# apirrone/Open_Duck_Playground

Measured on AMD Instinct MI355X. Metric: env-steps/sec open_duck_mini_v2 flat_terrain @8192 envs; 1/2/4/8-GPU scaling, higher is better.
Workload: dtype f32

## Files before the change

include/odk.h:

```cpp
#ifndef ODK_H
#define ODK_H

#include <stdint.h>

#ifdef __cplusplus
extern "C" {
#endif

typedef struct odk_model odk_model;
typedef struct odk_batch odk_batch;

enum odk_status {
  ODK_OK = 0,
  ODK_ERR_INVALID = -1,
  ODK_ERR_UNSUPPORTED = -2,
  ODK_ERR_HIP = -3,
  ODK_ERR_NOMEM = -4
};

#define ODK_NOBS 101
#define ODK_NPRIV 212
#define ODK_NOBS_STANDING 85
#define ODK_NPRIV_STANDING 153
#define ODK_ENV_JOYSTICK 0
// ... 28 lines not shown
  float* metrics_dev;
} odk_outputs;

enum odk_param {
  ODK_PARAM_BODY_MASS = 0,
  ODK_PARAM_BODY_IPOS_TORSO = 1,
  ODK_PARAM_DOF_FRICTIONLOSS = 2,
  ODK_PARAM_DOF_ARMATURE = 3,
  ODK_PARAM_QPOS0 = 4,
  ODK_PARAM_KP = 5
};

const char* odk_last_error(void);
void odk_default_config(odk_env_config* cfg);
void odk_default_config_standing(odk_env_config* cfg);
void odk_obs_sizes(int env_kind, int* nobs, int* npriv);

int odk_model_load(const void* blob, uint64_t len, odk_model** out);
void odk_model_free(odk_model* m);
int odk_model_dims(const odk_model* m, int* nq, int* nv, int* nu, int* nbody);
int odk_model_obs_sizes(const odk_model* m, int env_kind, int* nobs, int* npriv);

int odk_model_reduced(const odk_model* m, int* paired, int* nvr, int* nMr, int* nHr, int* red_main, int* red_twin);
int odk_model_env_lds_floats(const odk_model* m);

int odk_batch_create(const odk_model* m, const odk_env_config* cfg, int nenv, int device, const float* prm_table,
                     const double* dxs, int nx, const double* dys, int ny, const double* dths, int nth, const double* ranges6,
                     int nsteps_in_period, odk_batch** out);
void odk_batch_destroy(odk_batch* b);
int odk_batch_set_config(odk_batch* b, const odk_env_config* cfg);

int odk_batch_set_param(odk_batch* b, int param, const float* host_values, int count_per_env);

int odk_reset(odk_batch* b, uint32_t seed, uint32_t env_id_offset, const odk_outputs* outs, void* stream);

int odk_step(odk_batch* b, const float* action_dev, const odk_outputs* outs, void* stream);

int odk_batch_bind_commands(odk_batch* b, const float* cmd_dev, int row_stride);

#define ODK_NXTERM 12
enum odk_xterm {
  ODK_XTERM_LIN_VEL_Z = 0, ODK_XTERM_ANG_VEL_XY = 1, ODK_XTERM_ORIENTATION = 2, ODK_XTERM_BASE_HEIGHT = 3, ODK_XTERM_ENERGY = 4,
  ODK_XTERM_JOINT_POS_LIMITS = 5, ODK_XTERM_TERMINATION = 6, ODK_XTERM_POSE = 7, ODK_XTERM_FEET_SLIP = 8, ODK_XTERM_FEET_CLEARANCE = 9,
  ODK_XTERM_FEET_HEIGHT = 10, ODK_XTERM_FEET_AIR_TIME = 11
};
typedef struct {
// ... 148 lines not shown
```

open_duck_playground_amd/csrc/odk_engine.hip:

```cpp
#include <hip/hip_runtime.h>
#include <stddef.h>

#include <cmath>
#include <cstdarg>
#include <cstdio>
#include <cstdlib>
#include <cstring>
#include <array>
#include <string>
#include <vector>

#include "../../include/odk.h"
#include "odk_kernels.h"

using namespace odk;

struct RecLay {
  int CMD, LAST, LAST2, LAST3, MT, AIR, PEAK, PUSH, AHIST, IMU, EPSTEPS, TRUNC, DONE, EPSUM, EPLEN, EPMET, KEY0, KEY1, CTR, STEP, PSTEP, PINT, IMI, LCON, NINFO;
};
constexpr RecLay rec_lay(int nu) {
  RecLay r{};
  r.CMD = 0; r.LAST = 7; r.LAST2 = r.LAST + nu; r.LAST3 = r.LAST2 + nu; r.MT = r.LAST3 + nu; r.AIR = r.MT + nu; r.PEAK = r.AIR + 2; r.PUSH = r.PEAK + 2;
  r.AHIST = r.PUSH + 2; r.IMU = r.AHIST + 3 * nu; r.EPSTEPS = r.IMU + 9; r.TRUNC = r.EPSTEPS + 1; r.DONE = r.TRUNC + 1; r.EPSUM = r.DONE + 1; r.EPLEN = r.EPSUM + 1;
  r.EPMET = r.EPLEN + 1; r.KEY0 = r.EPMET + ODK_NMETRIC; r.KEY1 = r.KEY0 + 1; r.CTR = r.KEY1 + 1; r.STEP = r.CTR + 1; r.PSTEP = r.STEP + 1; r.PINT = r.PSTEP + 1;
// ... 920 lines not shown
  if (solref[1] <= 0) b = -solref[1] / dmax;
  P[0] = k; P[1] = b; P[2] = dmin; P[3] = dmax; P[4] = 1.0f / width; P[5] = mid; P[6] = power;
  P[7] = 1.0f / powf(mid, power - 1.0f); P[8] = 1.0f / powf(1.0f - mid, power - 1.0f);
}

namespace {
struct SparseLayout { int depth[MAXV], adr[MAXV], ancmask[MAXV], descmask[MAXV], anc_at[MAXV][MAXV], nnz; };
void sparse_layout(const int* parent, int n, SparseLayout& L) {
  L.nnz = 0;
  for (int i = 0; i < n; i++) {
    L.depth[i] = parent[i] < 0 ? 0 : L.depth[parent[i]] + 1;
    L.adr[i] = L.nnz; L.nnz += L.depth[i] + 1;
    L.ancmask[i] = 0; L.descmask[i] = 0;
  }
  for (int i = 0; i < n; i++) {
    int a = i;
    for (int c = L.depth[i]; c >= 0; c--, a = parent[a]) {
      L.anc_at[i][c] = a;
      if (a != i) { L.ancmask[i] |= 1 << a; L.descmask[a] |= 1 << i; }
    }
  }
}
}
static void fill_body_st(DevModel& m) {
  auto fill = [&](BodySt& b, int bi, bool in) {
    memset(&b, 0, sizeof(b));
    b.level = in ? m.body_level[bi] : -2;
    b.parent = m.body_parent[bi];
    b.nchild = in ? m.body_nchild[bi] : 0;
    b.pathmask = in ? m.body_pathmask[bi] : 0;
    b.is_path = in ? m.body_is_path[bi] : 0;
    b.upmask = in ? m.body_upmask[bi] : 0;
    b.path_head = in ? m.body_path_head[bi] : 0;
    for (int k = 0; k < 3; k++) b.child[k] = m.body_children[bi][k];
    b.njnt = (in && b.level > 0) ? m.body_jntnum[bi] : 0;
    for (int k = 0; k < 2; k++) {
      const bool on = k < b.njnt;
      const int j = on ? m.body_jntadr[bi] + k : 0;
      b.jj[k] = j;
      b.jd[k] = m.jnt_dofadr[j];
      b.jr[k] = (m.paired && m.dof_tkind[b.jd[k]] == 2) ? -1 : m.dof_red[b.jd[k]];
      for (int c = 0; c < 3; c++) b.ax[k][c] = on ? m.jnt_axis[j][c] : 0.0f;
    }
    for (int c = 0; c < 3; c++) { b.pos[c] = m.body_pos[bi][c]; b.ipos[c] = m.body_ipos[bi][c]; }
    for (int c = 0; c < 4; c++) b.quat[c] = m.body_quat[bi][c];
    for (int c = 0; c < 6; c++) b.inertia[c] = m.body_inertia[bi][c];
  };
  for (int bi = 0; bi < m.nb; bi++) fill(m.body_st[bi], bi, true);
  fill(m.body_st[MAXB], 0, false);
}

static bool build_reduced_tables(DevModel& m) {
  m.paired = 0; m.nrchain = 0;
  int ntwin = 0;
  for (int d = 0; d < MAXV; d++) { m.dof_tkind[d] = 0; m.dof_red[d] = 0; m.red_main[d] = 0; m.red_twin[d] = -1; }
  for (int v = 7; v < m.nv; v++) {
    const int u = v - 1, ju = m.dof_jnt[u], jv = m.dof_jnt[v];
    if (ju < 0 || jv < 0 || m.dof_tkind[u] != 0) continue;
    const bool same = m.dof_body[u] == m.dof_body[v] && m.dof_anc[v][1] == u && m.jnt_axis[ju][0] == m.jnt_axis[jv][0] &&
                      m.jnt_axis[ju][1] == m.jnt_axis[jv][1] && m.jnt_axis[ju][2] == m.jnt_axis[jv][2];
    if (!same) continue;
    m.dof_tkind[u] = 1; m.dof_tkind[v] = 2; ntwin++;
  }
  m.paired = ntwin > 0;
  int nr = 0;
  for (int d = 0; d < m.nv; d++) {
    if (m.dof_tkind[d] == 2) { m.dof_red[d] = m.dof_red[d - 1]; continue; }
    m.dof_red[d] = nr; m.red_main[nr] = d; m.red_twin[nr] = m.dof_tkind[d] == 1 ? d + 1 : -1; nr++;
  }
  m.nvr = nr;
  int rparent[MAXV], rvparent[MAXV];
  for (int r = 0; r < nr; r++) {
// ... 431 lines not shown
  if (eulerdamp != 0 || m.iterations != 1) { delete mo; return fail(ODK_ERR_UNSUPPORTED, "kernels implement iterations=1, eulerdamp=disable (open_duck_mini_v2.xml:6-8)"); }
  for (int s = 0; s < m.nsensor; s++) {
    int b = m.site_body[m.sensor_site[s]];
    bool ok = (b == m.base_body) || (b == m.foot_body[0]) || (b == m.foot_body[1]);
    if (!ok || ((m.sensor_type[s] == 2 || m.sensor_type[s] == 8) && b != m.base_body)) { delete mo; return fail(ODK_ERR_UNSUPPORTED, "sensor %d placement", s); }
  }
  m.np_count = 0;
  for (int b2 = 0; b2 < m.nb; b2++) {
    if (!(m.body_level[b2] >= 0 && m.body_nchild[b2] > 0 && !m.body_is_path[b2])) continue;
    if (m.np_count == 4) { delete mo; return fail(ODK_ERR_UNSUPPORTED, "more than four branching bodies above the serial chains"); }
    const int i = m.np_count++;
    m.np_body[i] = b2; m.np_nsrc[i] = 0;
    for (int c2 = 0; c2 < m.nb; c2++) {
      bool below = false;
      for (int a2 = c2; a2 > 0; a2 = m.body_parent[a2]) if (a2 == b2) { below = true; break; }
      if (!below || m.body_level[c2] < 0) continue;
      if (!m.body_is_path[c2] || m.body_path_head[c2]) {
        if (m.np_nsrc[i] == 6) { delete mo; return fail(ODK_ERR_UNSUPPORTED, "more than six sources in a subtree fold"); }
        m.np_src[i][m.np_nsrc[i]++] = c2;
      }
    }
  }
  if (!build_reduced_tables(m)) { delete mo; return fail(ODK_ERR_UNSUPPORTED, "dof tree is not a floating base with up to three serial chains of <= 5 (twin-merged) dofs"); }
  fill_body_st(m);
  int dt_max = 0, dv_max = 0;
  for (int d = 0; d < m.nv; d++) { dt_max = m.dof_depth[d] > dt_max ? m.dof_depth[d] : dt_max; dv_max = m.vdof_depth[d] > dv_max ? m.vdof_depth[d] : dv_max; }
  mo->shape = -1;
#define X(i, S) if (mo->shape < 0 && m.nq == S::NQ && m.nv == S::NV && m.nb == S::NB && m.nu == S::NU && m.nj == S::NJ && m.nM == S::NM && m.nH == S::NH && m.nrow == S::NROW && \
                    dt_max <= S::DT && dv_max <= S::DV) mo->shape = i;
  ODK_SHAPES(X)
#undef X
  if (mo->shape < 0) {
    const int dtm = dt_max, dvm = dv_max;
    delete mo;
    return fail(ODK_ERR_UNSUPPORTED, "model shape nq=%d nv=%d nb=%d nu=%d nj=%d nM=%d nH=%d nrow=%d depth=%d vdepth=%d has no compiled kernel (tools/new_shape.py <xml> prints the two lines to add to odk_engine.hip)",
                m.nq, m.nv, m.nb, m.nu, m.nj, m.nM, m.nH, m.nrow, dtm, dvm);
  }
  int shape_cl = 5; bool shape_eq = false;
#define X(i, S) if (mo->shape == i) { shape_cl = S::CL; shape_eq = S::EQ; }
  ODK_SHAPES(X)
#undef X
  for (int c = 0; c < m.nrchain; c++)
    if (m.rchain_len[c] > shape_cl) { const int len = m.rchain_len[c]; delete mo; return fail(ODK_ERR_UNSUPPORTED, "a serial chain of %d (twin-merged) dofs: the kernels of this model shape solve chains of <= %d", len, shape_cl); }
  if (!m.floor_is_plane && mo->shape != 1) { delete mo; return fail(ODK_ERR_UNSUPPORTED, "height-field floors are built for the backlash model only"); }

  if (m.cone && m.foot_prim != 0) {
    delete mo; return fail(ODK_ERR_UNSUPPORTED, "<option cone=\"elliptic\">: the elliptic-cone kernels are built for convex (box / mesh) feet, not sphere / capsule feet");
// ... 87 lines not shown
}
extern "C" void odk_model_free(odk_model* m) { delete m; }
extern "C" int odk_model_dims(const odk_model* m, int* nq, int* nv, int* nu, int* nbody) {
  if (!m) return fail(ODK_ERR_INVALID, "null model");
  if (nq) *nq = m->h.nq; if (nv) *nv = m->h.nv; if (nu) *nu = m->h.nu; if (nbody) *nbody = m->h.nb;
  return ODK_OK;
}
extern "C" int odk_model_obs_sizes(const odk_model* m, int env_kind, int* nobs, int* npriv) {
  if (!m) return fail(ODK_ERR_INVALID, "null model");
  obs_sizes_nu(m->h.nu, env_kind, nobs, npriv);
  return ODK_OK;
}

#ifndef ODK_PROFILE
static_assert(EnvL<ShapeA>::wg_floats(2) * sizeof(float) <= 20480, "shape A: LDS image too large for 8 workgroups per CU");
static_assert(EnvL<ShapeB>::wg_floats(2) * sizeof(float) <= 20480, "shape B: LDS image too large for 8 workgroups per CU");
#endif
extern "C" int odk_model_reduced(const odk_model* m, int* paired, int* nvr, int* nMr, int* nHr, int* red_main, int* red_twin) {
  if (!m) return fail(ODK_ERR_INVALID, "null model");
  if (paired) *paired = m->h.paired; if (nvr) *nvr = m->h.nvr; if (nMr) *nMr = m->h.nMr; if (nHr) *nHr = m->h.nHr;
  for (int r = 0; r < m->h.nvr; r++) { if (red_main) red_main[r] = m->h.red_main[r]; if (red_twin) red_twin[r] = m->h.red_twin[r]; }
  return ODK_OK;
}
extern "C" int odk_model_env_lds_floats(const odk_model* m) {
  if (!m) return -1;
#define X(i, S) if (m->shape == i) return EnvL<S>::TOTAL;
  ODK_SHAPES(X)
#undef X
  return -1;
}

template <class S> static void fill_sizes(odk_batch* b) {
  b->rec_size = Rec<S>::SIZE; b->frec_size = Rec<S>::FSIZE; b->lds_total = S::TOTAL; b->dr_size = DRL<S>::SIZE; b->env_lds = EnvL<S>::TOTAL;
}

static void to_dev_cfg(const odk_env_config& c, EnvCfg& d, int nu) {
  d.ctrl_dt = c.ctrl_dt; d.action_scale = c.action_scale; d.dof_vel_scale = c.dof_vel_scale; d.max_motor_velocity = c.max_motor_velocity;
  d.noise_level = c.noise_level; d.noise_gyro = c.noise_gyro; d.noise_accelerometer = c.noise_accelerometer; d.noise_gravity = c.noise_gravity;
  d.noise_joint_vel = c.noise_joint_vel;
  memcpy(d.qpos_noise_scale, c.qpos_noise_scale, sizeof(d.qpos_noise_scale)); memcpy(d.reward_scales, c.reward_scales, sizeof(d.reward_scales));
  d.tracking_sigma = c.tracking_sigma; d.push_enable = c.push_enable;
  memcpy(d.push_interval_range, c.push_interval_range, 8); memcpy(d.push_magnitude_range, c.push_magnitude_range, 8);
  memcpy(d.cmd_range, c.cmd_range, sizeof(d.cmd_range));
  d.use_imitation = c.use_imitation; d.use_motor_speed_limits = c.use_motor_speed_limits; d.autoreset = c.autoreset;
  d.episode_length = c.episode_length; d.n_substeps = c.n_substeps;
  d.kind = c.env_kind; d.reset_base_qvel = c.reset_base_qvel;
// ... 454 lines not shown
```

open_duck_playground_amd/csrc/odk_kernels.h:

```cpp
#pragma once
#include <hip/hip_runtime.h>

#include "odk_model.h"

namespace odk {

#define ODK_SYNC() asm volatile("" ::: "memory")

constexpr float MINVAL_F = 1e-15f;
constexpr float PI_F = 3.14159265358979323846f;

struct EnvCfg {
  float ctrl_dt, action_scale, dof_vel_scale, max_motor_velocity;
  float noise_level, noise_gyro, noise_accelerometer, noise_gravity, noise_joint_vel;
  float qpos_noise_scale[16];
  float reward_scales[7];
  float tracking_sigma;
  float push_enable, push_interval_range[2], push_magnitude_range[2];
  float cmd_range[7][2];
  int use_imitation, use_motor_speed_limits, autoreset, episode_length, n_substeps;
  int kind, nobs, npriv;
  float reset_base_qvel;
};

// ... 92 lines not shown
#endif

#define ODK_DPP(v, ctrl, rmask) __int_as_float(__builtin_amdgcn_update_dpp(0, __float_as_int(v), ctrl, rmask, 0xF, true))
struct OpSum { static __device__ __forceinline__ float f(float a, float b) { return a + b; } };
struct OpMax { static __device__ __forceinline__ float f(float a, float b) { return fmaxf(a, b); } };
struct OpMin { static __device__ __forceinline__ float f(float a, float b) { return fminf(a, b); } };
typedef unsigned int odk_u2 __attribute__((ext_vector_type(2)));
template <int G, class Op> __device__ __forceinline__ float greduce(float v) {
  v = Op::f(v, ODK_DPP(v, 0xB1, 0xF));
  v = Op::f(v, ODK_DPP(v, 0x4E, 0xF));
  v = Op::f(v, ODK_DPP(v, 0x141, 0xF));
  v = Op::f(v, ODK_DPP(v, 0x140, 0xF));
  const unsigned iv = __float_as_uint(v);
  const odk_u2 h = __builtin_amdgcn_permlane16_swap(iv, iv, false, false);
  v = Op::f(__uint_as_float(h[0]), __uint_as_float(h[1]));
  if (G == 64) {
    const unsigned iw = __float_as_uint(v);
    const odk_u2 w = __builtin_amdgcn_permlane32_swap(iw, iw, false, false);
    v = Op::f(__uint_as_float(w[0]), __uint_as_float(w[1]));
  }
  return v;
}
template <int G> __device__ __forceinline__ float gsum(float v) { return greduce<G, OpSum>(v); }
template <int G, int N> __device__ __forceinline__ void gsum_n(float* v) {
  if constexpr (G == 32) {
    float o[N];
#pragma unroll
    for (int i = 0; i < N; i++) {
      float x = v[i];
      x += ODK_DPP(x, 0xB1, 0xF); x += ODK_DPP(x, 0x4E, 0xF); x += ODK_DPP(x, 0x141, 0xF); x += ODK_DPP(x, 0x140, 0xF);
      v[i] = x;
      o[i] = __int_as_float(__builtin_amdgcn_ds_swizzle(__float_as_int(x), 0x401F));
    }
#pragma unroll
    for (int i = 0; i < N; i++) v[i] += o[i];
  } else {
#pragma unroll
    for (int i = 0; i < N; i++) v[i] = gsum<G>(v[i]);
  }
}
__device__ __forceinline__ unsigned fkey(float v) { const unsigned b = __float_as_uint(v); return b ^ ((b >> 31) ? 0xFFFFFFFFu : 0x80000000u); }
__device__ __forceinline__ float fkey_inv(unsigned k) { return __uint_as_float(k ^ ((k >> 31) ? 0x80000000u : 0xFFFFFFFFu)); }
#define ODK_DPPU(v, ctrl) ((unsigned)__builtin_amdgcn_update_dpp(0, (int)(v), ctrl, 0xF, 0xF, true))
template <int G, bool MAX> __device__ __forceinline__ unsigned greduce_u(unsigned v) {
  auto op = [](unsigned a, unsigned b) { return MAX ? (a > b ? a : b) : (a < b ? a : b); };
  v = op(v, ODK_DPPU(v, 0xB1));
// ... 144 lines not shown
      for (int h = 0; h < 2; h++) {
        const int j = 2 * jp + h;
        int off = S::O_CDOF * 4;
        if (j < S::NVR && ((rel >> j) & 1)) off = (S::O_M + (j < r ? st.r_Madr + m->red_depth[j] : m->red_Madr[j] + st.r_depth)) * 4;
        pk |= off << (16 * h);
      }
      st.m_adr[jp] = pk;
    }
  }
  const int i = lane < S::NV ? lane : 0;
  st.d_on = lane < S::NV;
  st.d_body = m->dof_body[i];
  st.d_act = st.d_on ? m->dof_act[i] : -1;
  st.d_flrow = st.d_on ? m->dof_flrow[i] : -1;
  st.d_limrow = st.d_on ? m->dof_limrow[i] : -1;
  st.d_foot = st.d_on ? (m->foot_dofmask[0][i] | (m->foot_dofmask[1][i] << 1)) : 0;
  st.d_damping = m->dof_damping[i];
  st.d_lim_on = st.d_limrow >= 0;
  st.d_qadr = m->dof_qadr[i];
  st.d_lo = m->dof_range[i][0]; st.d_hi = m->dof_range[i][1];
  st.d_tkind = (S::PAIRED && st.d_on) ? m->dof_tkind[i] : 0;
  st.d_red = S::PAIRED ? m->dof_red[i] : i;
}
template <class S>
__device__ __forceinline__ void load_body(BodySt& b, const DevModel* __restrict__ m, int lane) {
  b = m->body_st[lane < S::NB ? lane : MAXB];
}
__device__ __forceinline__ void load_act(ActSt& a, const DevModel* __restrict__ m, int act) {
  const int u = act >= 0 ? act : 0;
  a.bias2 = m->act_bias2[u]; a.clo = m->act_ctrlrange[u][0]; a.chi = m->act_ctrlrange[u][1];
  a.flo = m->act_forcerange[u][0]; a.fhi = m->act_forcerange[u][1];
  a.climited = m->act_ctrllimited[u]; a.flimited = m->act_forcelimited[u];
}
__device__ __forceinline__ void load_fl(FlSt& f, const DevModel* __restrict__ m, int lane) {
  const int r = lane < m->nfl ? lane : 0;
  f.D = m->fl_D[r]; f.R = m->fl_R[r]; f.b = m->fl_b[r]; f.dof = m->fl_dof[r];
}
template <class S, int G>
__device__ __forceinline__ void load_hot(HotSt& h, const DevModel* __restrict__ m, const Statics<S, G>& st, int lane) {
  load_act(h.as, m, st.d_act);
  load_fl(h.fs, m, lane);
  const int f = (lane >> 4) & 1, j = lane & 15;
  const int jv = (lane < 32 && j < m->foot_nvert[f]) ? j : 0;
  for (int k = 0; k < 3; k++) h.vb[k] = m->foot_vert[f][jv][k];
}
__device__ __forceinline__ int load_rent(const DevModel* __restrict__ m, int p, int n) { const int e = m->R_ent[p < n ? p : 0]; return p < n ? e : -1; }
__device__ __forceinline__ int load_rhent(const DevModel* __restrict__ m, int p, int n) { const int e = m->RH_ent[p < n ? p : 0]; return p < n ? e : -1; }

template <int G, int DMAX, int NVT>
// ... 1254 lines not shown
}

template <class S, int G, int HF, bool PRE = false>
__device__ __forceinline__ void forward_env(float* L, const int* RT, const DevModel* __restrict__ m, const float* __restrict__ hfield, const Statics<S, G>& st, int lane, int flags, const HotSt& hot = HotSt()) {
  const float* SH = reinterpret_cast<const float*>(RT);
  const float* CT = SH + S::SH_CT;
  constexpr int NV = S::NV, NB = S::NB, NR = S::NVR;
  using ST = Statics<S, G>;
  float* QPOS = L + S::O_QPOS; float* QVEL = L + S::O_QVEL; float* WARM = L + S::O_WARM; float* CTRL = L + S::O_CTRL;
  float* Q0 = L + S::O_Q0; float* MASS = L + S::O_MASS; float* ARM = L + S::O_ARM; float* FRL = L + S::O_FRL; float* KP = L + S::O_KP;
  float* XPOS = L + S::O_XPOS; float* XQUAT = L + S::O_XQUAT; float* CVEL = L + S::O_CVEL; float* CACC = L + S::O_CACC;
  float* CFRC = L + S::O_CFRC; float* CRB = L + S::O_CRB; float* SC = L + S::O_SC; float* CDOF = L + S::O_CDOF;
  float* BUF6 = L + S::O_BUF6; float* BUF6B = L + S::O_BUF6B; float* M = L + S::O_M; float* HL = L + S::O_HL;
  float* QFS = L + S::O_QFS; float* QAS = L + S::O_QAS; float* X = L + S::O_X; float* MA = L + S::O_MA; float* GRAD = L + S::O_GRAD;
  float* MV = L + S::O_MV; float* ED = L + S::O_D; float* AREF = L + S::O_AREF; float* JAR = L + S::O_JAR; float* JV = L + S::O_JV;
  float* W = L + S::O_W; float* CDIST = L + S::O_CDIST; float* CR = L + S::O_CR; float* SCR = L + S::O_SCR;
  float* SENS = L + S::O_SENS; float* ACTF = L + S::O_ACTF;
  const int nfl = m->nfl, nlim = m->nlim, r0c = nfl + nlim;
  const float dt = m->dt;
  const float ref[3] = {QPOS[0], QPOS[1], QPOS[2]};
  ODK_PROF_BEGIN();

  BodySt bs;
  load_body<S>(bs, m, lane);
  if (st.j_qadr >= 0) {
    float s, c;
    const float x = 0.5f * (QPOS[st.j_qadr] - Q0[st.j_qadr]);
    if (fabsf(x) <= 1.7f) {
      const float x2 = x * x;
      float ps = 1.6059043836821613e-10f, pc = -1.1470745597729725e-11f;
      ps = fmaf(ps, x2, -2.505210838544172e-08f); pc = fmaf(pc, x2, 2.08767569878681e-09f);
      ps = fmaf(ps, x2, 2.7557319223985893e-06f); pc = fmaf(pc, x2, -2.755731922398589e-07f);
      ps = fmaf(ps, x2, -0.0001984126984126984f); pc = fmaf(pc, x2, 2.48015873015873e-05f);
      ps = fmaf(ps, x2, 0.008333333333333333f); pc = fmaf(pc, x2, -0.001388888888888889f);
      ps = fmaf(ps, x2, -0.16666666666666666f); pc = fmaf(pc, x2, 0.041666666666666664f);
      ps = fmaf(ps, x2, 1.0f); pc = fmaf(pc, x2, -0.5f);
      s = ps * x; c = fmaf(pc, x2, 1.0f);
    } else {
      sincosf(x, &s, &c);
    }
    SC[2 * lane] = s; SC[2 * lane + 1] = c;
  }
  ODK_SYNC();
  ODK_PROF(0);
  {
    float p[3] = {0, 0, 0}, q[4] = {1, 0, 0, 0}, cvel[6] = {0, 0, 0, 0, 0, 0}, cacc[6] = {0, 0, 0, 0, 0, 0};
    if (bs.level == -1) {
// ... 35 lines not shown
            if (jj < bs.njnt) {
              float axw[3], cd[6], dot[6];
              qrot(axw, q, bs.ax[jj]);
              const float off[3] = {ref[0] - p[0], ref[1] - p[1], ref[2] - p[2]};
              cd[0] = axw[0]; cd[1] = axw[1]; cd[2] = axw[2];
              cross3(cd + 3, axw, off);
              const int d = bs.jd[jj], col = bs.jr[jj];
              if (col >= 0) {
#pragma unroll
                for (int k = 0; k < 6; k++) CDOF[k * NR + col] = cd[k];
              }
              const float qv = QVEL[d];
              cross_motion(dot, cvel, cd);
#pragma unroll
              for (int k = 0; k < 6; k++) { cacc[k] += dot[k] * qv; cvel[k] += cd[k] * qv; }
              const float s = SC[2 * bs.jj[jj]], c = SC[2 * bs.jj[jj] + 1];
              const float qj[4] = {c, s * bs.ax[jj][0], s * bs.ax[jj][1], s * bs.ax[jj][2]};
              qmul(q, q, qj);
            }
          }
          qnormalize(q);
        }
#pragma unroll
        for (int k = 0; k < 3; k++) XPOS[k * NB + lane] = p[k];
#pragma unroll
        for (int k = 0; k < 4; k++) XQUAT[k * NB + lane] = q[k];
#pragma unroll
        for (int k = 0; k < 6; k++) { CVEL[k * NB + lane] = cvel[k]; CACC[k * NB + lane] = cacc[k]; }
      }
      ODK_SYNC();
    }
    {
      const bool isp = bs.is_path != 0, head = bs.path_head != 0;
      float ql[4] = {bs.quat[0], bs.quat[1], bs.quat[2], bs.quat[3]}, qb[2][4];
#pragma unroll
      for (int jj = 0; jj < 2; jj++) {
#pragma unroll
        for (int k = 0; k < 4; k++) qb[jj][k] = ql[k];
        if (jj < bs.njnt) {
          const float s = SC[2 * bs.jj[jj]], c = SC[2 * bs.jj[jj] + 1];
          const float qj[4] = {c, s * bs.ax[jj][0], s * bs.ax[jj][1], s * bs.ax[jj][2]};
          qmul(ql, ql, qj);
        }
      }
      float tp[3] = {bs.pos[0], bs.pos[1], bs.pos[2]}, tq[4] = {ql[0], ql[1], ql[2], ql[3]};
      float ppq[4] = {1, 0, 0, 0}, pcv[6] = {0, 0, 0, 0, 0, 0}, pca[6] = {0, 0, 0, 0, 0, 0};
      if (isp && head) {
        const int pb = bs.parent;
        float pp[3], t[3];
        for (int k = 0; k < 3; k++) pp[k] = XPOS[k * NB + pb];
        for (int k = 0; k < 4; k++) ppq[k] = XQUAT[k * NB + pb];
        for (int k = 0; k < 6; k++) { pcv[k] = CVEL[k * NB + pb]; pca[k] = CACC[k * NB + pb]; }
        qrot(t, ppq, tp);
        tp[0] = pp[0] + t[0]; tp[1] = pp[1] + t[1]; tp[2] = pp[2] + t[2];
        qmul(tq, ppq, tq);
      }
#pragma unroll
      for (int si = 0; si < 3; si++) {
        float up[3], uq[4];
#pragma unroll
        for (int k = 0; k < 3; k++) up[k] = __shfl_up(tp[k], 1 << si, G);
#pragma unroll
        for (int k = 0; k < 4; k++) uq[k] = __shfl_up(tq[k], 1 << si, G);
        if ((bs.upmask >> si) & 1) {
          float t[3];
          qrot(t, uq, tp);
          tp[0] = up[0] + t[0]; tp[1] = up[1] + t[1]; tp[2] = up[2] + t[2];
          qmul(tq, uq, tq);
        }
      }
      {
        float uq[4];
#pragma unroll
        for (int k = 0; k < 4; k++) uq[k] = __shfl_up(tq[k], 1, G);
        if (isp && !head) { ppq[0] = uq[0]; ppq[1] = uq[1]; ppq[2] = uq[2]; ppq[3] = uq[3]; }
      }
      float cd[2][6], qv[2] = {0, 0}, cinc[6] = {0, 0, 0, 0, 0, 0};
#pragma unroll
      for (int jj = 0; jj < 2; jj++) {
#pragma unroll
        for (int k = 0; k < 6; k++) cd[jj][k] = 0.0f;
        if (isp && jj < bs.njnt) {
          float qw[4], axw[3];
          qmul(qw, ppq, qb[jj]);
          qrot(axw, qw, bs.ax[jj]);
          const float off[3] = {ref[0] - tp[0], ref[1] - tp[1], ref[2] - tp[2]};
          cd[jj][0] = axw[0]; cd[jj][1] = axw[1]; cd[jj][2] = axw[2];
          cross3(cd[jj] + 3, axw, off);
          const int d = bs.jd[jj], col = bs.jr[jj];
          if (col >= 0) {
#pragma unroll
            for (int k = 0; k < 6; k++) CDOF[k * NR + col] = cd[jj][k];
          }
          qv[jj] = QVEL[d];
#pragma unroll
          for (int k = 0; k < 6; k++) cinc[k] += cd[jj][k] * qv[jj];
        }
      }
      float cv[6];
#pragma unroll
      for (int k = 0; k < 6; k++) cv[k] = cinc[k] + pcv[k];
#pragma unroll
      for (int si = 0; si < 3; si++) {
        float u[6];
#pragma unroll
        for (int k = 0; k < 6; k++) u[k] = __shfl_up(cv[k], 1 << si, G);
        const bool ok = (bs.upmask >> si) & 1;
#pragma unroll
        for (int k = 0; k < 6; k++) cv[k] += ok ? u[k] : 0.0f;
      }
      {
        float u[6];
#pragma unroll
        for (int k = 0; k < 6; k++) u[k] = __shfl_up(cv[k], 1, G);
        if (isp && !head) {
#pragma unroll
          for (int k = 0; k < 6; k++) pcv[k] = u[k];
        }
      }
      float ca[6];
#pragma unroll
      for (int k = 0; k < 6; k++) ca[k] = pca[k];
      if (isp) {
        float vb[6] = {pcv[0], pcv[1], pcv[2], pcv[3], pcv[4], pcv[5]};
#pragma unroll
        for (int jj = 0; jj < 2; jj++) {
          if (jj < bs.njnt) {
            float dot[6];
            cross_motion(dot, vb, cd[jj]);
#pragma unroll
            for (int k = 0; k < 6; k++) { ca[k] += dot[k] * qv[jj]; vb[k] += cd[jj][k] * qv[jj]; }
          }
        }
      }
#pragma unroll
      for (int si = 0; si < 3; si++) {
        float u[6];
#pragma unroll
        for (int k = 0; k < 6; k++) u[k] = __shfl_up(ca[k], 1 << si, G);
        const bool ok = (bs.upmask >> si) & 1;
#pragma unroll
        for (int k = 0; k < 6; k++) ca[k] += ok ? u[k] : 0.0f;
      }
      if (isp) {
        qnormalize(tq);
#pragma unroll
        for (int k = 0; k < 3; k++) { p[k] = tp[k]; XPOS[k * NB + lane] = tp[k]; }
#pragma unroll
        for (int k = 0; k < 4; k++) { q[k] = tq[k]; XQUAT[k * NB + lane] = tq[k]; }
#pragma unroll
        for (int k = 0; k < 6; k++) { cvel[k] = cv[k]; cacc[k] = ca[k]; CVEL[k * NB + lane] = cv[k]; CACC[k * NB + lane] = ca[k]; }
      }
      ODK_SYNC();
    }
    float acc[16];
#pragma unroll
    for (int k = 0; k < 16; k++) acc[k] = 0.0f;
    if (lane < NB) {
      if (bs.level < 0) {
#pragma unroll
        for (int k = 0; k < 3; k++) XPOS[k * NB + lane] = p[k];
#pragma unroll
        for (int k = 0; k < 4; k++) XQUAT[k * NB + lane] = q[k];
#pragma unroll
        for (int k = 0; k < 6; k++) { CVEL[k * NB + lane] = 0; CACC[k * NB + lane] = 0; }
      }
      float R[9];
      q2mat(R, q);
      float ip[3] = {bs.ipos[0], bs.ipos[1], bs.ipos[2]};
      {
        const float i0 = L[S::O_IPOS1], i1 = L[S::O_IPOS1 + 1], i2 = L[S::O_IPOS1 + 2];
        asm volatile("" :: "v"(i0), "v"(i1), "v"(i2));
        ip[0] = lane == 1 ? i0 : ip[0]; ip[1] = lane == 1 ? i1 : ip[1]; ip[2] = lane == 1 ? i2 : ip[2];
      }
      float off[3];
      for (int k = 0; k < 3; k++) off[k] = p[k] + R[3 * k] * ip[0] + R[3 * k + 1] * ip[1] + R[3 * k + 2] * ip[2] - ref[k];
      const float* f = bs.inertia;
      const float Ib[9] = {f[0], f[3], f[4], f[3], f[1], f[5], f[4], f[5], f[2]};
      float T[9], Iw[9];
      for (int i = 0; i < 3; i++)
        for (int j = 0; j < 3; j++) T[3 * i + j] = R[3 * i] * Ib[j] + R[3 * i + 1] * Ib[3 + j] + R[3 * i + 2] * Ib[6 + j];
      for (int i = 0; i < 3; i++)
        for (int j = 0; j < 3; j++) Iw[3 * i + j] = T[3 * i] * R[3 * j] + T[3 * i + 1] * R[3 * j + 1] + T[3 * i + 2] * R[3 * j + 2];
      const float mb = MASS[lane], o2 = dot3(off, off);
      float ci[10];
      ci[0] = Iw[0] + mb * (o2 - off[0] * off[0]);
      ci[1] = Iw[4] + mb * (o2 - off[1] * off[1]);
      ci[2] = Iw[8] + mb * (o2 - off[2] * off[2]);
      ci[3] = Iw[1] - mb * off[0] * off[1];
      ci[4] = Iw[2] - mb * off[0] * off[2];
      ci[5] = Iw[5] - mb * off[1] * off[2];
      ci[6] = mb * off[0]; ci[7] = mb * off[1]; ci[8] = mb * off[2];
      ci[9] = mb;
      float fr[6], t1[6], a3[3], c3[3];
      inert_mul(fr, ci, cacc);
      inert_mul(t1, ci, cvel);
      cross3(a3, cvel, t1);
      cross3(c3, cvel + 3, t1 + 3);
      fr[0] += a3[0] + c3[0]; fr[1] += a3[1] + c3[1]; fr[2] += a3[2] + c3[2];
      cross3(a3, cvel, t1 + 3);
      fr[3] += a3[0]; fr[4] += a3[1]; fr[5] += a3[2];
      const bool dyn = bs.level >= 0;
#pragma unroll
      for (int k = 0; k < 10; k++) acc[k] = dyn ? ci[k] : 0.0f;
#pragma unroll
      for (int k = 0; k < 6; k++) acc[10 + k] = dyn ? fr[k] : 0.0f;
    }
    ODK_PROF(1);
#pragma unroll
    for (int si = 0; si < 3; si++) {
      const bool ok = (bs.pathmask >> si) & 1;
      float t[16];
#pragma unroll
      for (int k = 0; k < 16; k++) t[k] = __shfl_down(acc[k], 1 << si, G);
#pragma unroll
      for (int k = 0; k < 16; k++) acc[k] += ok ? t[k] : 0.0f;
    }
    if (lane < NB) {
#pragma unroll
      for (int k = 0; k < 10; k++) CRB[k * NB + lane] = acc[k];
#pragma unroll
      for (int k = 0; k < 6; k++) CFRC[k * NB + lane] = acc[10 + k];
    }
    ODK_SYNC();
  }
  {
    float* ACC = CFRC;
    static_assert(S::O_CRB == S::O_CFRC + 6 * NB, "cfrc | crb must be contiguous");
    const int nnp = m->np_count;
    const int slot = lane >> 4, q = lane & 15;
    float t[2] = {0.0f, 0.0f};
#pragma unroll
    for (int pass = 0; pass < 2; pass++) {
      const int i = pass * (G / 16) + slot;
      if (i < nnp) {
        const int ns = m->np_nsrc[i];
        int src[6];
#pragma unroll
        for (int c = 0; c < 6; c++) src[c] = m->np_src[i][c];
        float x = 0.0f;
#pragma unroll
        for (int c = 0; c < 6; c++) { const float y = ACC[q * NB + src[c]]; x += c < ns ? y : 0.0f; }
        t[pass] = x;
      }
    }
// ... 1133 lines not shown
```

open_duck_playground_amd/csrc/odk_model.h:

```cpp
#pragma once
#include <stdint.h>

namespace odk {

constexpr int EQ_MAX = 2;
constexpr int EQP_MAX = 2, EQP_ROWS = 9;
constexpr int MAXV = 32;
constexpr int MAXQ = 32;
constexpr int MAXB = 20;
constexpr int MAXJ = 26;
constexpr int MAXU = 16;
constexpr int MAXNZ = 512;
constexpr int MAXHV = 20;
constexpr int MAXHF = 40;
constexpr int MAXHE = 64;
constexpr int HULL_MAXV = 17;
constexpr int HULL_MAXF = 30;
constexpr int HULL_MAXE = 48;
static_assert(HULL_MAXV <= MAXHV && HULL_MAXF <= MAXHF && HULL_MAXE <= MAXHE && HULL_MAXF <= 32 && HULL_MAXE <= 48 && HULL_MAXV <= 17, "kernel hull regions");
constexpr int MAXCHAIN = 8;
constexpr int MAXSITE = 8;
constexpr int MAXSENS = 16;
constexpr int NCON = 12;
constexpr int NSENSD = 46;

struct BodySt {
  int level, parent, nchild, child[3], njnt, jd[2], jj[2], jr[2], pathmask, is_path, upmask, path_head;
  float pos[3], quat[4], ipos[3], inertia[6], ax[2][3];
  int pad;
};

struct LaneSt {
  int j_qadr, j_dadr;
  int cs_pk;
  int ch_first, ch_len;
  int r_on, r_depth, r_Madr, r_ancmask, r_descmask, r_foot;
  int m_adr[16];
  int d_on, d_body;
  int d_act, d_flrow, d_limrow, d_foot;
  int d_qadr, d_lim_on;
  int d_tkind, d_red;
  float d_damping, d_lo, d_hi;
};

struct DevModel {
  BodySt body_st[MAXB + 1];
  LaneSt lane_st[64];
  int nq, nv, nu, nb, nj, nM, nH, nfl, nlim, nrow, nsite, nsensor;
  float dt, gravity[3], tolerance, ls_tolerance, impratio, meaninertia;
  int ls_iterations, iterations;
  int base_body, body_in_tree[MAXB], body_parent[MAXB], body_jntadr[MAXB], body_jntnum[MAXB];
  int max_level, body_level[MAXB], body_children[MAXB][3], body_nchild[MAXB];
  int max_nonpath_level, body_pathmask[MAXB], body_is_path[MAXB], body_upmask[MAXB], body_path_head[MAXB];
  int np_count, np_body[4], np_nsrc[4], np_src[4][MAXB];
  int body_chain[MAXB][MAXCHAIN], body_chain_len[MAXB];
  int body_ancdof[MAXB][MAXV], body_nancdof[MAXB];
  int body_sub[MAXB][MAXB], body_nsub[MAXB];
  float body_pos[MAXB][3], body_quat[MAXB][4], body_ipos[MAXB][3], body_mass[MAXB], body_inertia[MAXB][6];
  int jnt_qposadr[MAXJ], jnt_dofadr[MAXJ], jnt_bodyid[MAXJ];
  float jnt_axis[MAXJ][3], jnt_pos[MAXJ][3], jnt_range[MAXJ][2], qpos0[MAXQ];
  int dof_body[MAXV], dof_depth[MAXV], dof_anc[MAXV][MAXV], dof_Madr[MAXV], dof_anc_adr[MAXV][MAXV];
  int dof_ndesc[MAXV], dof_desc[MAXV][MAXV], dof_desc_adr[MAXV][MAXV];
  int dof_nprefix[MAXV], dof_prefix[MAXV][MAXV];
  int dof_nsym[MAXV], dof_sym_dof[MAXV][MAXV], dof_sym_adr[MAXV][MAXV];
  int dof_act[MAXV], dof_flrow[MAXV], dof_limrow[MAXV];
  int dof_ancmask[MAXV], dof_descmask[MAXV], vdof_ancmask[MAXV], vdof_descmask[MAXV];
  int dof_qadr[MAXV], dof_jnt[MAXV];
  float dof_range[MAXV][2];
  float dof_armature[MAXV], dof_damping[MAXV], dof_frictionloss[MAXV], dof_invweight0[MAXV];
// ... 88 lines not shown
```

open_duck_playground_amd/engine.py:

```python
from __future__ import annotations

import ctypes as C
import os
import subprocess
from typing import Dict, Optional

import numpy as np

from .model import Model, asset_path

_CSRC = os.path.join(os.path.dirname(os.path.abspath(__file__)), "csrc")
LIB_PATH = os.environ.get("ODK_LIB", os.path.join(_CSRC, "libodk.so"))

NOBS, NPRIV, NMETRIC, NU = 101, 212, 8, 14
ADAM_ACC_FLOATS = 2 + 1024
METRIC_NAMES = ("reward/tracking_lin_vel", "reward/tracking_ang_vel", "cost/torques", "cost/action_rate", "cost/stand_still",
                "reward/alive", "reward/imitation", "swing_peak")

XTERM_NAMES = ("lin_vel_z", "ang_vel_xy", "orientation", "base_height", "energy", "joint_pos_limits", "termination", "pose", "feet_slip",
               "feet_clearance", "feet_height", "feet_air_time")
NXTERM = len(XTERM_NAMES)

PARAM_BODY_MASS, PARAM_BODY_IPOS_TORSO, PARAM_DOF_FRICTIONLOSS, PARAM_DOF_ARMATURE, PARAM_QPOS0, PARAM_KP = range(6)


class EnvConfig(C.Structure):
    _fields_ = [
        ("ctrl_dt", C.c_float), ("action_scale", C.c_float), ("dof_vel_scale", C.c_float), ("max_motor_velocity", C.c_float),
# ... 70 lines not shown


def load_library() -> C.CDLL:
    global _lib
    if _lib is not None:
        return _lib
    if not os.path.exists(LIB_PATH):
        raise OdkError(f"{LIB_PATH} is missing: run `python -c 'import __graft_entry__ as g; g.build()'` "
                       "(there is no CPU fallback for the env engine)")
    import torch
    L = C.CDLL(LIB_PATH)
    P, PP = C.c_void_p, C.POINTER(C.c_void_p)
    FP, DP = C.POINTER(C.c_float), C.POINTER(C.c_double)
    L.odk_last_error.restype = C.c_char_p
    L.odk_default_config.argtypes = [C.POINTER(EnvConfig)]
    L.odk_default_config_standing.argtypes = [C.POINTER(EnvConfig)]
    L.odk_obs_sizes.argtypes = [C.c_int, C.POINTER(C.c_int), C.POINTER(C.c_int)]
    L.odk_model_load.argtypes = [C.c_char_p, C.c_uint64, PP]
    L.odk_model_free.argtypes = [P]
    L.odk_model_dims.argtypes = [P] + [C.POINTER(C.c_int)] * 4
    L.odk_model_obs_sizes.argtypes = [P, C.c_int, C.POINTER(C.c_int), C.POINTER(C.c_int)]
    L.odk_batch_lanes.argtypes = [P]
    L.odk_model_reduced.argtypes = [P] + [C.POINTER(C.c_int)] * 6
    L.odk_model_env_lds_floats.argtypes = [P]
    L.odk_batch_create.argtypes = [P, C.POINTER(EnvConfig), C.c_int, C.c_int, FP, DP, C.c_int, DP, C.c_int, DP, C.c_int, DP, C.c_int, PP]
    L.odk_batch_destroy.argtypes = [P]
    L.odk_batch_set_config.argtypes = [P, C.POINTER(EnvConfig)]
    L.odk_batch_set_param.argtypes = [P, C.c_int, FP, C.c_int]
    L.odk_reset.argtypes = [P, C.c_uint32, C.c_uint32, C.POINTER(Outputs), P]
    L.odk_step.argtypes = [P, P, C.POINTER(Outputs), P]
    L.odk_physics_step.argtypes = [P, P, C.c_int, P]
    L.odk_batch_bind_commands.argtypes = [P, P, C.c_int]
    L.odk_batch_set_reward_terms.argtypes = [P, C.POINTER(RewardTerms)]
    L.odk_batch_bind_reward_metrics.argtypes = [P, P]
    L.odk_tracking_accumulate.argtypes = [P, P, P, P, P, P, P]
    L.odk_batch_get_state.argtypes = [P, FP, FP, FP]
    L.odk_batch_set_state.argtypes = [P, FP, FP, FP]
    L.odk_batch_get_debug.argtypes = [P, FP, FP, FP, FP]
    L.odk_set_debug_dump.argtypes = [C.c_int]
    L.odk_batch_lds_size.argtypes = [P]
    L.odk_batch_get_lds.argtypes = [P, FP]
    L.odk_lds_offset.argtypes = [P, C.c_char_p]
    L.odk_batch_record_size.argtypes = [P]
    L.odk_batch_get_records.argtypes = [P, FP]
    L.odk_batch_set_records.argtypes = [P, FP]
    L.odk_batch_timing.argtypes = [P, C.c_int, FP, C.POINTER(C.c_int)]
# ... 6 lines not shown
    L.odk_colsum_partial.argtypes = [P, P, C.c_int, C.c_int, P]
    L.odk_colsum_finalize.argtypes = [PP, PP, C.POINTER(C.c_int), C.c_int, C.c_int, P]
    L.odk_dw_gemm.argtypes = [PP, PP, C.POINTER(C.c_int), C.POINTER(C.c_int), C.POINTER(C.c_longlong), C.c_int, C.POINTER(C.c_int), C.c_int, P, C.c_longlong, P,
                              C.POINTER(GradFinish), P]
    IP, LP = C.POINTER(C.c_int), C.POINTER(C.c_longlong)
    L.odk_mlp_forward.argtypes = [C.POINTER(MlpDesc), C.c_int, P]
    L.odk_mlp_backward.argtypes = [C.POINTER(MlpDesc), C.c_int, P]
    L.odk_mlp_set_profile.argtypes = [P]
    L.odk_mlp_set_profile.restype = None
    L.odk_pack_weights.argtypes = [P, C.c_longlong, P, C.c_longlong, P, C.c_longlong, C.POINTER(WeightTableC), P]
    L.odk_adam_clip_packed.argtypes = [P, P, P, P, P, C.c_longlong] + [C.c_float] * 5 + [P, C.c_longlong, P, C.c_longlong, C.POINTER(WeightTableC), C.c_int, P]
    L.odk_adam_clip_packed_tail.argtypes = [P, P, P, P, P, C.c_longlong] + [C.c_float] * 5 + [P, C.c_longlong, P, C.c_longlong, C.POINTER(WeightTableC), C.c_int,
                                            C.POINTER(StepTail), P]
    L.odk_ppo_gae_head.argtypes = [C.POINTER(GaeHeadArgs), P]
    L.odk_col_moments.argtypes = [P, C.c_longlong, C.c_int, C.c_int, P, P]
    L.odk_moments_update.argtypes = [P, C.c_int, C.c_int, C.c_longlong, P, P, P, P, C.c_float, C.c_float, P]
    L.odk_colsum_fold.argtypes = [PP, PP, IP, IP, C.c_int, P]
    L.odk_gather_rows.argtypes = [C.POINTER(C.c_void_p), C.POINTER(C.c_void_p), C.POINTER(C.c_int), C.POINTER(C.c_longlong), C.c_int, P, C.c_int, C.c_longlong, P]
    _lib = L
    return L


EXPORTED_SYMBOLS = (
    "odk_last_error", "odk_default_config", "odk_default_config_standing", "odk_obs_sizes", "odk_model_load", "odk_model_free", "odk_model_dims", "odk_model_obs_sizes", "odk_batch_lanes", "odk_model_reduced",
    "odk_model_env_lds_floats", "odk_batch_create",
    "odk_batch_destroy", "odk_batch_set_config", "odk_batch_set_param", "odk_reset", "odk_step", "odk_physics_step",
    "odk_batch_bind_commands", "odk_batch_set_reward_terms", "odk_batch_bind_reward_metrics", "odk_tracking_accumulate",
    "odk_batch_get_state", "odk_batch_set_state", "odk_batch_get_debug", "odk_set_debug_dump", "odk_batch_lds_size",
    "odk_batch_get_lds", "odk_lds_offset", "odk_batch_record_size", "odk_batch_get_records", "odk_batch_set_records", "odk_batch_timing", "odk_gae", "odk_ppo_head",
    "odk_policy_sample", "odk_adam_clip", "odk_silu_bwd_colsum", "odk_colsum_partial", "odk_colsum_finalize", "odk_gather_rows", "odk_dw_gemm",
    "odk_mlp_forward", "odk_mlp_backward", "odk_mlp_set_profile", "odk_pack_weights", "odk_adam_clip_packed", "odk_colsum_fold",
    "odk_adam_clip_packed_tail", "odk_ppo_gae_head", "odk_col_moments", "odk_moments_update")


TRACK_NACC = 12
TRACK_ENDED, TRACK_STEPS, TRACK_SAMPLES, TRACK_FALLS, TRACK_REWARD, TRACK_SUM, TRACK_SQERR = 0, 1, 2, 3, 4, 5, 8
NCOMMAND = 7


def check_commands(cmd, nenv: int, device: int) -> None:
    import torch
    if not torch.is_tensor(cmd):
        raise OdkError(f"commands: expected a torch tensor or None, got {type(cmd).__name__}")
    if tuple(cmd.shape) != (int(nenv), NCOMMAND):
        raise OdkError(f"commands: shape must be ({nenv}, {NCOMMAND}), got {tuple(cmd.shape)}")
    if cmd.dtype != torch.float32:
        raise OdkError(f"commands: dtype must be torch.float32, got {cmd.dtype}")
# ... 26 lines not shown
    blob = model.blob()
    h = C.c_void_p()
    _chk(L.odk_model_load(blob, len(blob), C.byref(h)))
    try:
        a, b = C.c_int(0), C.c_int(0)
        _chk(L.odk_model_obs_sizes(h, int(env_kind), C.byref(a), C.byref(b)))
        return a.value, b.value
    finally:
        L.odk_model_free(h)


def model_reduction(model: Model) -> Dict:
    L = load_library()
    blob = model.blob()
    h = C.c_void_p()
    _chk(L.odk_model_load(blob, len(blob), C.byref(h)))
    try:
        ints = [C.c_int(0) for _ in range(4)]
        main, twin = (C.c_int * 32)(), (C.c_int * 32)()
        _chk(L.odk_model_reduced(h, *[C.byref(i) for i in ints], main, twin))
        nvr = ints[1].value
        return dict(paired=ints[0].value, nvr=nvr, nMr=ints[2].value, nHr=ints[3].value, main=list(main)[:nvr], twin=list(twin)[:nvr],
                    env_lds_floats=L.odk_model_env_lds_floats(h))
    finally:
        L.odk_model_free(h)


def load_prm() -> Dict[str, np.ndarray]:
    z = np.load(asset_path("prm_table.npz"))
    return {k: z[k] for k in z.files}


def _fp(a: np.ndarray):
    return a.ctypes.data_as(C.POINTER(C.c_float))


def _dp(a: np.ndarray):
    return a.ctypes.data_as(C.POINTER(C.c_double))


def _stream(t):
    import torch
    return C.c_void_p(torch.cuda.current_stream(t.device).cuda_stream)


def _ptr(t):
# ... 613 lines not shown
```

Before: 19.05 million.

## Pack body chains into 16-lane rows and use DPP row shifts for scans

Builds a body-to-lane layout so each serial body chain sits within one 16-lane DPP row, and stores per-lane body tables for 32- and 64-lane groups. The kinematic and composite-inertia prefix scans then use DPP row_shr/row_shl instead of __shfl_up/__shfl_down, which avoids LDS-backed cross-lane permutes. Writes to per-body LDS arrays are indexed by the mapped body id instead of the lane. In exchange, models whose chains do not fit a 16-lane row are now rejected, and the quaternion/position scan computes both branches unconditionally before selecting.

```diff
diff --git a/include/odk.h b/include/odk.h
--- a/include/odk.h
+++ b/include/odk.h
@@ -74,6 +74,7 @@
 int odk_model_obs_sizes(const odk_model* m, int env_kind, int* nobs, int* npriv);
 
 int odk_model_reduced(const odk_model* m, int* paired, int* nvr, int* nMr, int* nHr, int* red_main, int* red_twin);
+int odk_model_body_lanes(const odk_model* m, int lanes_per_env, int* out, int n);
 int odk_model_env_lds_floats(const odk_model* m);
 
 int odk_batch_create(const odk_model* m, const odk_env_config* cfg, int nenv, int device, const float* prm_table,
diff --git a/open_duck_playground_amd/csrc/odk_engine.hip b/open_duck_playground_amd/csrc/odk_engine.hip
--- a/open_duck_playground_amd/csrc/odk_engine.hip
+++ b/open_duck_playground_amd/csrc/odk_engine.hip
@@ -966,7 +966,26 @@
   }
 }
 }
-static void fill_body_st(DevModel& m) {
+static bool build_body_lanes(const DevModel& m, int G, int* lane_body) {
+  for (int l = 0; l < 64; l++) lane_body[l] = -1;
+  for (int b = 0; b < m.nb; b++) {
+    if (m.body_is_path[b] && !m.body_path_head[b]) continue;
+    int len = 1;
+    if (m.body_is_path[b])
+      while (b + len < m.nb && m.body_is_path[b + len] && !m.body_path_head[b + len]) len++;
+    int at = -1;
+    for (int s = 0; s + len <= G && at < 0; s++) {
+      if ((s >> 4) != ((s + len - 1) >> 4)) continue;
+      bool free = true;
+      for (int k = 0; k < len; k++) free = free && lane_body[s + k] < 0;
+      if (free) at = s;
+    }
+    if (at < 0) return false;
+    for (int k = 0; k < len; k++) lane_body[at + k] = b + k;
+  }
+  return true;
+}
+static bool fill_body_st(DevModel& m) {
   auto fill = [&](BodySt& b, int bi, bool in) {
     memset(&b, 0, sizeof(b));
     b.level = in ? m.body_level[bi] : -2;
@@ -990,8 +1009,16 @@
     for (int c = 0; c < 4; c++) b.quat[c] = m.body_quat[bi][c];
     for (int c = 0; c < 6; c++) b.inertia[c] = m.body_inertia[bi][c];
   };
-  for (int bi = 0; bi < m.nb; bi++) fill(m.body_st[bi], bi, true);
-  fill(m.body_st[MAXB], 0, false);
+  for (int g = 0; g < 2; g++) {
+    int lane_body[64];
+    if (!build_body_lanes(m, g ? 64 : 32, lane_body)) return false;
+    for (int l = 0; l < 64; l++) {
+      const int bi = lane_body[l];
+      fill(m.body_st[g][l], bi >= 0 ? bi : 0, bi >= 0);
+      m.body_st[g][l].body = bi;
+    }
+  }
+  return true;
 }
 
 static bool build_reduced_tables(DevModel& m) {
@@ -1469,7 +1496,9 @@
     }
   }
   if (!build_reduced_tables(m)) { delete mo; return fail(ODK_ERR_UNSUPPORTED, "dof tree is not a floating base with up to three serial chains of <= 5 (twin-merged) dofs"); }
-  fill_body_st(m);
+  if (!fill_body_st(m)) {
+    delete mo; return fail(ODK_ERR_UNSUPPORTED, "no body-to-lane layout: every serial body chain must fit in one 16-lane row and all %d bodies in 32 lanes", m.nb);
+  }
   int dt_max = 0, dv_max = 0;
   for (int d = 0; d < m.nv; d++) { dt_max = m.dof_depth[d] > dt_max ? m.dof_depth[d] : dt_max; dv_max = m.vdof_depth[d] > dv_max ? m.vdof_depth[d] : dv_max; }
   mo->shape = -1;
@@ -1603,6 +1632,11 @@
   for (int r = 0; r < m->h.nvr; r++) { if (red_main) red_main[r] = m->h.red_main[r]; if (red_twin) red_twin[r] = m->h.red_twin[r]; }
   return ODK_OK;
 }
+extern "C" int odk_model_body_lanes(const odk_model* m, int lanes_per_env, int* out, int n) {
+  if (!m || !out || (lanes_per_env != 32 && lanes_per_env != 64)) return fail(ODK_ERR_INVALID, "odk_model_body_lanes: bad arguments");
+  for (int l = 0; l < n && l < lanes_per_env; l++) out[l] = m->h.body_st[lanes_per_env == 64][l].body;
+  return ODK_OK;
+}
 extern "C" int odk_model_env_lds_floats(const odk_model* m) {
   if (!m) return -1;
 #define X(i, S) if (m->shape == i) return EnvL<S>::TOTAL;
diff --git a/open_duck_playground_amd/csrc/odk_kernels.h b/open_duck_playground_amd/csrc/odk_kernels.h
--- a/open_duck_playground_amd/csrc/odk_kernels.h
+++ b/open_duck_playground_amd/csrc/odk_kernels.h
@@ -138,6 +138,8 @@
   return v;
 }
 template <int G> __device__ __forceinline__ float gsum(float v) { return greduce<G, OpSum>(v); }
+__device__ __forceinline__ float row_shr(float v, int si) { return si == 0 ? ODK_DPP(v, 0x111, 0xF) : si == 1 ? ODK_DPP(v, 0x112, 0xF) : ODK_DPP(v, 0x114, 0xF); }
+__device__ __forceinline__ float row_shl(float v, int si) { return si == 0 ? ODK_DPP(v, 0x101, 0xF) : si == 1 ? ODK_DPP(v, 0x102, 0xF) : ODK_DPP(v, 0x104, 0xF); }
 template <int G, int N> __device__ __forceinline__ void gsum_n(float* v) {
   if constexpr (G == 32) {
     float o[N];
@@ -328,9 +330,9 @@
   st.d_tkind = (S::PAIRED && st.d_on) ? m->dof_tkind[i] : 0;
   st.d_red = S::PAIRED ? m->dof_red[i] : i;
 }
-template <class S>
+template <int G>
 __device__ __forceinline__ void load_body(BodySt& b, const DevModel* __restrict__ m, int lane) {
-  b = m->body_st[lane < S::NB ? lane : MAXB];
+  b = m->body_st[G == 64][lane];
 }
 __device__ __forceinline__ void load_act(ActSt& a, const DevModel* __restrict__ m, int act) {
   const int u = act >= 0 ? act : 0;
@@ -1631,7 +1633,8 @@
   ODK_PROF_BEGIN();
 
   BodySt bs;
-  load_body<S>(bs, m, lane);
+  load_body<G>(bs, m, lane);
+  const int bid = bs.body;
   if (st.j_qadr >= 0) {
     float s, c;
     const float x = 0.5f * (QPOS[st.j_qadr] - Q0[st.j_qadr]);
@@ -1713,11 +1716,11 @@
           qnormalize(q);
         }
 #pragma unroll
-        for (int k = 0; k < 3; k++) XPOS[k * NB + lane] = p[k];
-#pragma unroll
-        for (int k = 0; k < 4; k++) XQUAT[k * NB + lane] = q[k];
-#pragma unroll
-        for (int k = 0; k < 6; k++) { CVEL[k * NB + lane] = cvel[k]; CACC[k * NB + lane] = cacc[k]; }
+        for (int k = 0; k < 3; k++) XPOS[k * NB + bid] = p[k];
+#pragma unroll
+        for (int k = 0; k < 4; k++) XQUAT[k * NB + bid] = q[k];
+#pragma unroll
+        for (int k = 0; k < 6; k++) { CVEL[k * NB + bid] = cvel[k]; CACC[k * NB + bid] = cacc[k]; }
       }
       ODK_SYNC();
     }
@@ -1750,20 +1753,22 @@
       for (int si = 0; si < 3; si++) {
         float up[3], uq[4];
 #pragma unroll
-        for (int k = 0; k < 3; k++) up[k] = __shfl_up(tp[k], 1 << si, G);
-#pragma unroll
-        for (int k = 0; k < 4; k++) uq[k] = __shfl_up(tq[k], 1 << si, G);
-        if ((bs.upmask >> si) & 1) {
-          float t[3];
-          qrot(t, uq, tp);
-          tp[0] = up[0] + t[0]; tp[1] = up[1] + t[1]; tp[2] = up[2] + t[2];
-          qmul(tq, uq, tq);
-        }
+        for (int k = 0; k < 3; k++) up[k] = row_shr(tp[k], si);
+#pragma unroll
+        for (int k = 0; k < 4; k++) uq[k] = row_shr(tq[k], si);
+        const bool ok = (bs.upmask >> si) & 1;
+        float t[3], nq[4];
+        qrot(t, uq, tp);
+        qmul(nq, uq, tq);
+#pragma unroll
+        for (int k = 0; k < 3; k++) tp[k] = ok ? up[k] + t[k] : tp[k];
+#pragma unroll
+        for (int k = 0; k < 4; k++) tq[k] = ok ? nq[k] : tq[k];
       }
       {
         float uq[4];
 #pragma unroll
-        for (int k = 0; k < 4; k++) uq[k] = __shfl_up(tq[k], 1, G);
+        for (int k = 0; k < 4; k++) uq[k] = row_shr(tq[k], 0);
         if (isp && !head) { ppq[0] = uq[0]; ppq[1] = uq[1]; ppq[2] = uq[2]; ppq[3] = uq[3]; }
       }
       float cd[2][6], qv[2] = {0, 0}, cinc[6] = {0, 0, 0, 0, 0, 0};
@@ -1793,17 +1798,14 @@
       for (int k = 0; k < 6; k++) cv[k] = cinc[k] + pcv[k];
 #pragma unroll
       for (int si = 0; si < 3; si++) {
-        float u[6];
-#pragma unroll
-        for (int k = 0; k < 6; k++) u[k] = __shfl_up(cv[k], 1 << si, G);
-        const bool ok = (bs.upmask >> si) & 1;
-#pragma unroll
-        for (int k = 0; k < 6; k++) cv[k] += ok ? u[k] : 0.0f;
+        const bool ok = (bs.pathmask >> si) & 1;
+#pragma unroll
+        for (int k = 0; k < 6; k++) cv[k] += row_shr(ok ? cv[k] : 0.0f, si);
       }
       {
         float u[6];
 #pragma unroll
-        for (int k = 0; k < 6; k++) u[k] = __shfl_up(cv[k], 1, G);
+        for (int k = 0; k < 6; k++) u[k] = row_shr(cv[k], 0);
         if (isp && !head) {
 #pragma unroll
           for (int k = 0; k < 6; k++) pcv[k] = u[k];
@@ -1826,35 +1828,32 @@
       }
 #pragma unroll
       for (int si = 0; si < 3; si++) {
-        float u[6];
-#pragma unroll
-        for (int k = 0; k < 6; k++) u[k] = __shfl_up(ca[k], 1 << si, G);
-        const bool ok = (bs.upmask >> si) & 1;
-#pragma unroll
-        for (int k = 0; k < 6; k++) ca[k] += ok ? u[k] : 0.0f;
+        const bool ok = (bs.pathmask >> si) & 1;
+#pragma unroll
+        for (int k = 0; k < 6; k++) ca[k] += row_shr(ok ? ca[k] : 0.0f, si);
       }
       if (isp) {
         qnormalize(tq);
 #pragma unroll
-        for (int k = 0; k < 3; k++) { p[k] = tp[k]; XPOS[k * NB + lane] = tp[k]; }
-#pragma unroll
-        for (int k = 0; k < 4; k++) { q[k] = tq[k]; XQUAT[k * NB + lane] = tq[k]; }
-#pragma unroll
-        for (int k = 0; k < 6; k++) { cvel[k] = cv[k]; cacc[k] = ca[k]; CVEL[k * NB + lane] = cv[k]; CACC[k * NB + lane] = ca[k]; }
+        for (int k = 0; k < 3; k++) { p[k] = tp[k]; XPOS[k * NB + bid] = tp[k]; }
+#pragma unroll
+        for (int k = 0; k < 4; k++) { q[k] = tq[k]; XQUAT[k * NB + bid] = tq[k]; }
+#pragma unroll
+        for (int k = 0; k < 6; k++) { cvel[k] = cv[k]; cacc[k] = ca[k]; CVEL[k * NB + bid] = cv[k]; CACC[k * NB + bid] = ca[k]; }
       }
       ODK_SYNC();
     }
     float acc[16];
 #pragma unroll
     for (int k = 0; k < 16; k++) acc[k] = 0.0f;
-    if (lane < NB) {
+    if (bid >= 0) {
       if (bs.level < 0) {
 #pragma unroll
-        for (int k = 0; k < 3; k++) XPOS[k * NB + lane] = p[k];
-#pragma unroll
-        for (int k = 0; k < 4; k++) XQUAT[k * NB + lane] = q[k];
-#pragma unroll
-        for (int k = 0; k < 6; k++) { CVEL[k * NB + lane] = 0; CACC[k * NB + lane] = 0; }
+        for (int k = 0; k < 3; k++) XPOS[k * NB + bid] = p[k];
+#pragma unroll
+        for (int k = 0; k < 4; k++) XQUAT[k * NB + bid] = q[k];
+#pragma unroll
+        for (int k = 0; k < 6; k++) { CVEL[k * NB + bid] = 0; CACC[k * NB + bid] = 0; }
       }
       float R[9];
       q2mat(R, q);
@@ -1862,7 +1861,7 @@
       {
         const float i0 = L[S::O_IPOS1], i1 = L[S::O_IPOS1 + 1], i2 = L[S::O_IPOS1 + 2];
         asm volatile("" :: "v"(i0), "v"(i1), "v"(i2));
-        ip[0] = lane == 1 ? i0 : ip[0]; ip[1] = lane == 1 ? i1 : ip[1]; ip[2] = lane == 1 ? i2 : ip[2];
+        ip[0] = bid == 1 ? i0 : ip[0]; ip[1] = bid == 1 ? i1 : ip[1]; ip[2] = bid == 1 ? i2 : ip[2];
       }
       float off[3];
       for (int k = 0; k < 3; k++) off[k] = p[k] + R[3 * k] * ip[0] + R[3 * k + 1] * ip[1] + R[3 * k + 2] * ip[2] - ref[k];
@@ -1873,7 +1872,7 @@
         for (int j = 0; j < 3; j++) T[3 * i + j] = R[3 * i] * Ib[j] + R[3 * i + 1] * Ib[3 + j] + R[3 * i + 2] * Ib[6 + j];
       for (int i = 0; i < 3; i++)
         for (int j = 0; j < 3; j++) Iw[3 * i + j] = T[3 * i] * R[3 * j] + T[3 * i + 1] * R[3 * j + 1] + T[3 * i + 2] * R[3 * j + 2];
-      const float mb = MASS[lane], o2 = dot3(off, off);
+      const float mb = MASS[bid], o2 = dot3(off, off);
       float ci[10];
       ci[0] = Iw[0] + mb * (o2 - off[0] * off[0]);
       ci[1] = Iw[4] + mb * (o2 - off[1] * off[1]);
@@ -1900,18 +1899,15 @@
     ODK_PROF(1);
 #pragma unroll
     for (int si = 0; si < 3; si++) {
-      const bool ok = (bs.pathmask >> si) & 1;
-      float t[16];
-#pragma unroll
-      for (int k = 0; k < 16; k++) t[k] = __shfl_down(acc[k], 1 << si, G);
-#pragma unroll
-      for (int k = 0; k < 16; k++) acc[k] += ok ? t[k] : 0.0f;
-    }
-    if (lane < NB) {
-#pragma unroll
-      for (int k = 0; k < 10; k++) CRB[k * NB + lane] = acc[k];
-#pragma unroll
-      for (int k = 0; k < 6; k++) CFRC[k * NB + lane] = acc[10 + k];
+      const bool ok = (bs.upmask >> si) & 1;
+#pragma unroll
+      for (int k = 0; k < 16; k++) acc[k] += row_shl(ok ? acc[k] : 0.0f, si);
+    }
+    if (bid >= 0) {
+#pragma unroll
+      for (int k = 0; k < 10; k++) CRB[k * NB + bid] = acc[k];
+#pragma unroll
+      for (int k = 0; k < 6; k++) CFRC[k * NB + bid] = acc[10 + k];
     }
     ODK_SYNC();
   }
diff --git a/open_duck_playground_amd/csrc/odk_model.h b/open_duck_playground_amd/csrc/odk_model.h
--- a/open_duck_playground_amd/csrc/odk_model.h
+++ b/open_duck_playground_amd/csrc/odk_model.h
@@ -27,7 +27,7 @@
 struct BodySt {
   int level, parent, nchild, child[3], njnt, jd[2], jj[2], jr[2], pathmask, is_path, upmask, path_head;
   float pos[3], quat[4], ipos[3], inertia[6], ax[2][3];
-  int pad;
+  int body;
 };
 
 struct LaneSt {
@@ -44,7 +44,7 @@
 };
 
 struct DevModel {
-  BodySt body_st[MAXB + 1];
+  BodySt body_st[2][64];
   LaneSt lane_st[64];
   int nq, nv, nu, nb, nj, nM, nH, nfl, nlim, nrow, nsite, nsensor;
   float dt, gravity[3], tolerance, ls_tolerance, impratio, meaninertia;
diff --git a/open_duck_playground_amd/engine.py b/open_duck_playground_amd/engine.py
--- a/open_duck_playground_amd/engine.py
+++ b/open_duck_playground_amd/engine.py
@@ -3,7 +3,7 @@
 import ctypes as C
 import os
 import subprocess
-from typing import Dict, Optional
+from typing import Dict, List, Optional
 
 import numpy as np
 
@@ -120,6 +120,7 @@
     L.odk_model_obs_sizes.argtypes = [P, C.c_int, C.POINTER(C.c_int), C.POINTER(C.c_int)]
     L.odk_batch_lanes.argtypes = [P]
     L.odk_model_reduced.argtypes = [P] + [C.POINTER(C.c_int)] * 6
+    L.odk_model_body_lanes.argtypes = [P, C.c_int, C.POINTER(C.c_int), C.c_int]
     L.odk_model_env_lds_floats.argtypes = [P]
     L.odk_batch_create.argtypes = [P, C.POINTER(EnvConfig), C.c_int, C.c_int, FP, DP, C.c_int, DP, C.c_int, DP, C.c_int, DP, C.c_int, PP]
     L.odk_batch_destroy.argtypes = [P]
@@ -172,7 +173,7 @@
 
 
 EXPORTED_SYMBOLS = (
-    "odk_last_error", "odk_default_config", "odk_default_config_standing", "odk_obs_sizes", "odk_model_load", "odk_model_free", "odk_model_dims", "odk_model_obs_sizes", "odk_batch_lanes", "odk_model_reduced",
+    "odk_last_error", "odk_default_config", "odk_default_config_standing", "odk_obs_sizes", "odk_model_load", "odk_model_free", "odk_model_dims", "odk_model_obs_sizes", "odk_batch_lanes", "odk_model_reduced", "odk_model_body_lanes",
     "odk_model_env_lds_floats", "odk_batch_create",
     "odk_batch_destroy", "odk_batch_set_config", "odk_batch_set_param", "odk_reset", "odk_step", "odk_physics_step",
     "odk_batch_bind_commands", "odk_batch_set_reward_terms", "odk_batch_bind_reward_metrics", "odk_tracking_accumulate",
@@ -245,6 +246,19 @@
         nvr = ints[1].value
         return dict(paired=ints[0].value, nvr=nvr, nMr=ints[2].value, nHr=ints[3].value, main=list(main)[:nvr], twin=list(twin)[:nvr],
                     env_lds_floats=L.odk_model_env_lds_floats(h))
+    finally:
+        L.odk_model_free(h)
+
+
+def model_body_lanes(model: Model, lanes_per_env: int) -> List[int]:
+    L = load_library()
+    blob = model.blob()
+    h = C.c_void_p()
+    _chk(L.odk_model_load(blob, len(blob), C.byref(h)))
+    try:
+        out = (C.c_int * lanes_per_env)()
+        _chk(L.odk_model_body_lanes(h, int(lanes_per_env), out, lanes_per_env))
+        return list(out)
     finally:
         L.odk_model_free(h)
 
```

Result: faster. 19.80 million, median of 6 (+3.9%).
